# AI4Science-WestlakeU/safediffcon

Measured on AMD Instinct MI355X. Metric: sampled control trajectories/sec (1000-step DDPM), higher is better.
Workload: dtype f32; 1 GPU; C4: 2D smoke Unet3D_with_Conv3D dim=64 (1,2,4) state (B,32,7,64,64), B=64 per GPU, guided 1000-step DDPM, conformal quantile on; batch_per_gpu=64, global_batch=64, step=U-Net + guidance + posterior update of the whole batch, one hipGraph replay, parallelism=batch-sharded x1, no data-path collective, conv_precision=fp32

## Files before the change

include/sdc.h:

```cpp
#ifndef SDC_H
#define SDC_H

#include <stddef.h>
#include <stdint.h>

#ifdef __cplusplus
extern "C" {
#endif

#define SDC_OK 0
#define SDC_EINVAL (-1)
#define SDC_EALIGN (-2)
#define SDC_EHIP (-3)
#define SDC_ENULL (-4)

int sdc_version(void);
int sdc_last_error(char* buf, size_t cap);

typedef struct SdcConvDesc {
    int32_t B, Cin0, Cin1, Cout;
    int32_t iD, iH, iW;
    int32_t oD, oH, oW;
    int32_t kD, kH, kW;
    int32_t sD, sH, sW;
// ... 128 lines not shown
int sdc_burgers_rollout(const float* u0, const float* f, float* traj, int N, int s, int Nt, int steps, int record_every,
                        float dt, float coef_transport, float d0, float d1, float d2, void* stream);


typedef struct SdcWgradDesc {
    int32_t B, M, N;
    int32_t oD, oH, oW;
    int32_t iD, iH, iW;
    int32_t kD, kH, kW;
    int32_t sD, sH, sW;
    int32_t pD, pH, pW;
    int32_t uD, uH, uW;
    int32_t precision;
    int64_t gs[5], xs[5];
} SdcWgradDesc;
size_t sdc_conv_wgrad_bytes(const SdcWgradDesc* d);
int sdc_conv_wgrad(const SdcWgradDesc* d, const float* g, const float* x, float* dw, float* dbias, void* work,
                   size_t work_bytes, void* stream);

#define SDC_F16_EXP_INTS 1025
int sdc_f16_grad_exponent(const float* g, int B, int C, int D, int H, int W, const int64_t* strides, int32_t* e, void* stream);

int sdc_conv_dgrad_f16(const SdcConvDesc* d, const float* g, const float* wp, const int32_t* e, float* dx, void* stream);

size_t sdc_conv_wgrad_f16_bytes(const SdcWgradDesc* d);
int sdc_conv_wgrad_f16(const SdcWgradDesc* d, const float* g, const float* x, const int32_t* e, float* dw, float* dbias, void* work,
                       size_t work_bytes, void* stream);
int sdc_conv_wgrad_describe(const SdcWgradDesc* d, char* name, size_t cap);

int sdc_conv_stem_f16_ok(const SdcConvDesc* d);
size_t sdc_pack_stem_f16_bytes(int Cout, int Cin, int kD, int kH, int kW);
int sdc_pack_stem_f16(const float* w, void* out, int Cout, int Cin, int kD, int kH, int kW, void* stream);
int sdc_conv_stem_f16(const SdcConvDesc* d, const float* x, const void* wh, const float* bias, float* y, void* stream);

int sdc_conv_stem_x3_ok(const SdcConvDesc* d);
size_t sdc_pack_stem_x3_bytes(int Cout, int Cin, int kD, int kH, int kW);
int sdc_pack_stem_x3(const float* w, void* out, int Cout, int Cin, int kD, int kH, int kW, void* stream);
int sdc_conv_stem_x3(const SdcConvDesc* d, const float* x, const void* wb, const float* bias, float* y, void* stream);

int sdc_conv_gemm_x3_ok(const SdcConvDesc* d);
size_t sdc_pack_gemm_x3_bytes(int Cout, int Cin, int kH, int kW);
int sdc_pack_gemm_x3(const float* wp, void* out, int Cout, int Cin, int kH, int kW, void* stream);
int sdc_conv_gemm_x3(const SdcConvDesc* d, const float* x, const void* wb, const float* bias, float* y, void* stream);

int sdc_conv_pw_x3_ok(const SdcConvDesc* d);
int sdc_conv_pw_x3(const SdcConvDesc* d, const float* x0, const float* x1, const float* wp, const float* bias, const float* residual,
                   float* y, void* stream);

int sdc_conv_wino3_x3_ok(const SdcConvDesc* d);
size_t sdc_pack_wino3_x3_bytes(int Cout, int Cin);
int sdc_pack_wino3_x3(const float* wp, void* out, int Cout, int Cin, void* stream);
int sdc_conv_wino3_x3(const SdcConvDesc* d, const float* x, const float* x1, const void* wb, const float* bias, float* y,
                      double* gn_parts, int gn_groups, void* stream);

size_t sdc_gn_silu_bwd_floats(int B, int C, int G, int64_t S);
int sdc_gn_silu_bwd(const float* h, const float* gy, const float* stats, const float* gamma, const float* beta,
                    const float* ss, int64_t ss_b_stride, float* rows, float* gh, float* dgamma, float* dbeta, float* dss,
                    int B, int C, int G, int64_t S, void* stream);

size_t sdc_chan_norm_bwd_parts(int B, int64_t S);
size_t sdc_chan_norm_bwd_bytes(int B, int C, int64_t S);
int sdc_chan_norm_bwd(const float* x, const float* gy, const float* g, float* gx, float* gpart, int B, int C, int64_t S,
                      int mode, float eps, void* stream);

size_t sdc_pack_conv_weight_floats(int Cout, int Cin, int kD, int kH, int kW, int precision);
int sdc_pack_conv_weight(const float* w, float* out, int Cout, int Cin, int kD, int kH, int kW, int precision, int flip, void* stream);

typedef struct SdcPackItem {
    const float* w;
    float* out;
    int Cout, Cin, kD, kH, kW, precision, flip;
    int co_sh, ci_sh, grid_x, grid_y, block0;
    unsigned tap_magic;
    int64_t n[5];
} SdcPackItem;
int sdc_pack_batch_plan(SdcPackItem* items, int n, int* total_blocks, int* lds_bytes);
int sdc_pack_batch_run(const SdcPackItem* items_dev, int n, int total_blocks, int lds_bytes, void* stream);

size_t sdc_attn_bwd_bytes(int outer, int inner, int heads, int ntok);
int sdc_attn_bwd(const float* qkv, const float* dout, const float* rot, const float* bias, float* dqkv, float* dbias, void* work,
                 int outer, int inner, int heads, int ntok, int64_t q_so, int64_t q_sc, int64_t q_si, int64_t q_st,
                 int64_t o_so, int64_t o_sc, int64_t o_si, int64_t o_st, void* stream);

size_t sdc_tattn_block_bwd_bytes(int outer, int inner);
int sdc_tattn_block_bwd(const float* x, const float* g_pre, const float* wqkv, const float* wo, const float* rot, const float* bias,
                        const float* dy, float* dx, float* dg, float* dwqkv, float* dwo, float* dbias, void* work,
                        int outer, int inner, int C, int ntok, int64_t so, int64_t sc, int64_t st, float eps, void* stream);
size_t sdc_linattn_bwd_bytes(int outer, int inner, int heads, int64_t n);
int sdc_linattn_bwd(const float* qkv, const float* dout, float* dqkv, void* work, int outer, int inner, int heads, int64_t n,
                    int64_t q_so, int64_t q_sc, int64_t q_si, int64_t o_so, int64_t o_sc, int64_t o_si, void* stream);

int sdc_act_bwd(const float* x, const float* gy, float* gx, int64_t n, int kind, void* stream);

int sdc_sumpool2(const float* g, float* gx, int64_t rows, int H, int W, int fh, int fw, void* stream);

int sdc_linear(const float* x, const float* w, const float* bias, float* y, int rows, int K, int M, int64_t x_stride,
               int64_t y_stride, void* stream);
int sdc_linear_dgrad(const float* gy, const float* w, float* gx, int rows, int K, int M, int64_t gy_stride, int64_t gx_stride,
                     void* stream);
int sdc_linear_wgrad(const float* gy, const float* x, float* gw, float* gbias, int rows, int K, int M, int64_t gy_stride,
                     int64_t x_stride, void* stream);

typedef struct {
    const void* ptr;
    int64_t nwords;
} SdcSpan;
// ... 87 lines not shown
```

safediffcon_amd/_lib.py:

```python
import ctypes as C
import os

_HERE = os.path.dirname(os.path.abspath(__file__))
LIB_PATH = os.path.join(_HERE, "libsdc_hip.so")

SDC_MODEL_BURGERS, SDC_MODEL_TOKAMAK, SDC_MODEL_SMOKE = 0, 1, 2

_f32p = C.c_void_p
_i32p = C.c_void_p
_stream = C.c_void_p
_i64 = C.c_int64


class SdcConvDesc(C.Structure):
    _fields_ = [(n, C.c_int32) for n in (
        "B", "Cin0", "Cin1", "Cout", "iD", "iH", "iW", "oD", "oH", "oW", "kD", "kH", "kW", "sD", "sH", "sW",
        "pD", "pH", "pW", "uD", "uH", "uW", "up_mode", "precision")] + [
        ("x0s", C.c_int64 * 5), ("x1s", C.c_int64 * 5), ("ys", C.c_int64 * 5), ("rs", C.c_int64 * 5)]


class SdcStepDesc(C.Structure):
    _fields_ = [(n, C.c_int32) for n in (
        "model", "B", "d0", "d1", "d2", "d3", "guide", "clip", "impose", "cond_idx", "pad_zero", "use_max",
        "has_wgt", "skip_draws", "ddim")] + [("_pad", C.c_int32), ("seed", C.c_uint64)]
# ... 71 lines not shown
    "sdc_linattn_block_f16_bytes": (C.c_size_t, [C.c_int, C.c_int, C.c_int, _i64]),
    "sdc_linattn_block_f16": (C.c_int, [_f32p, _f32p, _f32p, _f32p, C.c_void_p, _f32p, _f32p, C.c_void_p, _f32p, C.c_int, C.c_int,
                                        C.c_int, _i64, _i64, _i64, _i64, C.c_int, C.c_int, C.c_float, _stream]),
    "sdc_linattn_block_gn_f16": (C.c_int, [_f32p, _f32p, _f32p, _f32p, C.c_int, _f32p, _f32p, _f32p, _f32p, C.c_void_p, _f32p, _f32p,
                                           C.c_void_p, _f32p, C.c_int, C.c_int, C.c_int, _i64, _i64, _i64, _i64, C.c_int, C.c_int,
                                           C.c_float, _stream]),
    "sdc_linattn_block_f16_ok": (C.c_int, [C.c_int, _i64]),
    "sdc_tattn_block": (C.c_int, [_f32p, _f32p, _f32p, _f32p, _f32p, _f32p, _f32p, C.c_int, C.c_int, C.c_int, C.c_int,
                                  _i64, _i64, _i64, C.c_float, _stream]),
    "sdc_pack_tattn_f16_bytes": (C.c_size_t, []),
    "sdc_pack_tattn_f16": (C.c_int, [_f32p, _f32p, C.c_void_p, _stream]),
    "sdc_tattn_block_f16": (C.c_int, [_f32p, _f32p, C.c_void_p, _f32p, _f32p, _f32p, C.c_int, C.c_int, C.c_int, C.c_int,
                                      _i64, _i64, _i64, C.c_float, _stream]),
    "sdc_pack_tattn_x3_bytes": (C.c_size_t, []),
    "sdc_pack_tattn_x3": (C.c_int, [_f32p, _f32p, C.c_void_p, _stream]),
    "sdc_tattn_block_x3": (C.c_int, [_f32p, _f32p, C.c_void_p, _f32p, _f32p, _f32p, C.c_int, C.c_int, C.c_int, C.c_int,
                                     _i64, _i64, _i64, C.c_float, _stream]),
    "sdc_tattn_block_x3_ok": (C.c_int, [C.c_int, C.c_int, C.c_int]),
    "sdc_attn": (C.c_int, [_f32p, _f32p, _f32p, _f32p, C.c_int, C.c_int, C.c_int, C.c_int, _i64, _i64, _i64, _i64,
                           _i64, _i64, _i64, _i64, _stream]),
    "sdc_act": (C.c_int, [_f32p, _f32p, _i64, C.c_int, _stream]),
    "sdc_guide_reduce": (C.c_int, [C.POINTER(SdcStepDesc), _f32p, _f32p, _f32p, _i32p, _f32p, _f32p, _stream]),
    "sdc_step_update": (C.c_int, [C.POINTER(SdcStepDesc), _f32p, _f32p, _f32p, _f32p, _i32p, _i32p, _f32p, _i64,
                                  _f32p, _f32p, _f32p, _f32p, _f32p, _f32p, _f32p, _f32p, _stream]),
    "sdc_impose": (C.c_int, [C.POINTER(SdcStepDesc), _f32p, _f32p, _f32p, _f32p, _stream]),
    "sdc_randn": (C.c_int, [_f32p, _i64, C.c_uint64, _i32p, _stream]),
    "sdc_advance": (C.c_int, [_i32p, C.c_int, _i32p, C.c_int, _stream]),
    "sdc_advance_table": (C.c_int, [_i32p, _i32p, _i32p, _i32p, C.c_int, _stream]),
    "sdc_conformal_score": (C.c_int, [C.POINTER(SdcStepDesc), _f32p, _f32p, _f32p, _f32p, _f32p, _f32p, _stream]),
    "sdc_burgers_rollout": (C.c_int, [_f32p, _f32p, _f32p, C.c_int, C.c_int, C.c_int, C.c_int, C.c_int, C.c_float, C.c_float,
                                      C.c_float, C.c_float, C.c_float, _stream]),
    "sdc_conv_wgrad_bytes": (C.c_size_t, [C.POINTER(SdcWgradDesc)]),
    "sdc_conv_wgrad": (C.c_int, [C.POINTER(SdcWgradDesc), _f32p, _f32p, _f32p, _f32p, C.c_void_p, C.c_size_t, _stream]),
    "sdc_f16_grad_exponent": (C.c_int, [_f32p, C.c_int, C.c_int, C.c_int, C.c_int, C.c_int, C.c_void_p, C.c_void_p, _stream]),
    "sdc_conv_dgrad_f16": (C.c_int, [C.POINTER(SdcConvDesc), _f32p, _f32p, C.c_void_p, _f32p, _stream]),
    "sdc_conv_stem_f16_ok": (C.c_int, [C.POINTER(SdcConvDesc)]),
    "sdc_pack_stem_f16_bytes": (C.c_size_t, [C.c_int, C.c_int, C.c_int, C.c_int, C.c_int]),
    "sdc_pack_stem_f16": (C.c_int, [_f32p, C.c_void_p, C.c_int, C.c_int, C.c_int, C.c_int, C.c_int, _stream]),
    "sdc_conv_stem_f16": (C.c_int, [C.POINTER(SdcConvDesc), _f32p, C.c_void_p, _f32p, _f32p, _stream]),
    "sdc_conv_stem_x3_ok": (C.c_int, [C.POINTER(SdcConvDesc)]),
    "sdc_pack_stem_x3_bytes": (C.c_size_t, [C.c_int, C.c_int, C.c_int, C.c_int, C.c_int]),
    "sdc_pack_stem_x3": (C.c_int, [_f32p, C.c_void_p, C.c_int, C.c_int, C.c_int, C.c_int, C.c_int, _stream]),
    "sdc_conv_stem_x3": (C.c_int, [C.POINTER(SdcConvDesc), _f32p, C.c_void_p, _f32p, _f32p, _stream]),
    "sdc_conv_gemm_x3_ok": (C.c_int, [C.POINTER(SdcConvDesc)]),
    "sdc_pack_gemm_x3_bytes": (C.c_size_t, [C.c_int, C.c_int, C.c_int, C.c_int]),
    "sdc_pack_gemm_x3": (C.c_int, [_f32p, C.c_void_p, C.c_int, C.c_int, C.c_int, C.c_int, _stream]),
    "sdc_conv_gemm_x3": (C.c_int, [C.POINTER(SdcConvDesc), _f32p, C.c_void_p, _f32p, _f32p, _stream]),
    "sdc_conv_pw_x3_ok": (C.c_int, [C.POINTER(SdcConvDesc)]),
    "sdc_conv_pw_x3": (C.c_int, [C.POINTER(SdcConvDesc), _f32p, _f32p, _f32p, _f32p, _f32p, _f32p, _stream]),
    "sdc_conv_wino3_x3_ok": (C.c_int, [C.POINTER(SdcConvDesc)]),
    "sdc_pack_wino3_x3_bytes": (C.c_size_t, [C.c_int, C.c_int]),
    "sdc_pack_wino3_x3": (C.c_int, [_f32p, C.c_void_p, C.c_int, C.c_int, _stream]),
    "sdc_conv_wino3_x3": (C.c_int, [C.POINTER(SdcConvDesc), _f32p, _f32p, C.c_void_p, _f32p, _f32p, C.c_void_p, C.c_int, _stream]),
    "sdc_conv_wgrad_f16_bytes": (C.c_size_t, [C.POINTER(SdcWgradDesc)]),
    "sdc_conv_wgrad_f16": (C.c_int, [C.POINTER(SdcWgradDesc), _f32p, _f32p, C.c_void_p, _f32p, _f32p, C.c_void_p, C.c_size_t, _stream]),
    "sdc_conv_wgrad_describe": (C.c_int, [C.POINTER(SdcWgradDesc), C.c_char_p, C.c_size_t]),
    "sdc_gn_silu_bwd_floats": (C.c_size_t, [C.c_int, C.c_int, C.c_int, _i64]),
    "sdc_gn_silu_bwd": (C.c_int, [_f32p, _f32p, _f32p, _f32p, _f32p, _f32p, _i64, _f32p, _f32p, _f32p, _f32p, _f32p,
                                  C.c_int, C.c_int, C.c_int, _i64, _stream]),
    "sdc_chan_norm_bwd_parts": (C.c_size_t, [C.c_int, _i64]),
    "sdc_chan_norm_bwd_bytes": (C.c_size_t, [C.c_int, C.c_int, _i64]),
    "sdc_chan_norm_bwd": (C.c_int, [_f32p, _f32p, _f32p, _f32p, _f32p, C.c_int, C.c_int, _i64, C.c_int, C.c_float, _stream]),
    "sdc_pack_conv_weight_floats": (C.c_size_t, [C.c_int, C.c_int, C.c_int, C.c_int, C.c_int, C.c_int]),
    "sdc_pack_conv_weight": (C.c_int, [_f32p, _f32p, C.c_int, C.c_int, C.c_int, C.c_int, C.c_int, C.c_int, C.c_int, _stream]),
    "sdc_pack_batch_plan": (C.c_int, [C.POINTER(SdcPackItem), C.c_int, C.POINTER(C.c_int), C.POINTER(C.c_int)]),
    "sdc_pack_batch_run": (C.c_int, [C.c_void_p, C.c_int, C.c_int, C.c_int, _stream]),
    "sdc_tattn_block_bwd_bytes": (C.c_size_t, [C.c_int, C.c_int]),
    "sdc_tattn_block_bwd": (C.c_int, [_f32p, _f32p, _f32p, _f32p, _f32p, _f32p, _f32p, _f32p, _f32p, _f32p, _f32p, _f32p, C.c_void_p,
                                      C.c_int, C.c_int, C.c_int, C.c_int, _i64, _i64, _i64, C.c_float, _stream]),
    "sdc_attn_bwd_bytes": (C.c_size_t, [C.c_int, C.c_int, C.c_int, C.c_int]),
    "sdc_attn_bwd": (C.c_int, [_f32p, _f32p, _f32p, _f32p, _f32p, _f32p, C.c_void_p, C.c_int, C.c_int, C.c_int, C.c_int,
                               _i64, _i64, _i64, _i64, _i64, _i64, _i64, _i64, _stream]),
    "sdc_linattn_bwd_bytes": (C.c_size_t, [C.c_int, C.c_int, C.c_int, _i64]),
    "sdc_linattn_bwd": (C.c_int, [_f32p, _f32p, _f32p, C.c_void_p, C.c_int, C.c_int, C.c_int, _i64, _i64, _i64, _i64, _i64, _i64, _i64,
                                  _stream]),
    "sdc_act_bwd": (C.c_int, [_f32p, _f32p, _f32p, _i64, C.c_int, _stream]),
    "sdc_sumpool2": (C.c_int, [_f32p, _f32p, _i64, C.c_int, C.c_int, C.c_int, C.c_int, _stream]),
    "sdc_kstar_lstm_floats": (C.c_size_t, []),
    "sdc_kstar_rollout": (C.c_int, [C.POINTER(SdcKstarModel), _f32p, _i64, _i64, _i64, C.c_void_p, C.c_void_p, C.c_int, C.c_int, _stream]),
    "sdc_smoke_rollout_workspace_bytes": (C.c_size_t, [C.c_int]),
    "sdc_smoke_rollout": (C.c_int, [_f32p, _f32p, _i64, _i64, _f32p, _i64, _f32p, _i64, C.c_void_p, C.c_void_p, C.c_void_p,
                                    C.c_int, C.c_int, C.c_void_p, C.c_void_p, C.c_void_p, C.c_size_t, C.c_int, C.c_int, C.c_int,
                                    C.c_int, C.c_int, C.c_int, C.c_double, C.c_int, _stream]),
    "sdc_conv_splitk_bytes": (C.c_size_t, [C.POINTER(SdcConvDesc)]),
    "sdc_conv_splitk": (C.c_int, [C.POINTER(SdcConvDesc), _f32p, _f32p, _f32p, _f32p, _f32p, _f32p, C.c_size_t, _stream]),
    "sdc_linear": (C.c_int, [_f32p, _f32p, _f32p, _f32p, C.c_int, C.c_int, C.c_int, _i64, _i64, _stream]),
    "sdc_linear_dgrad": (C.c_int, [_f32p, _f32p, _f32p, C.c_int, C.c_int, C.c_int, _i64, _i64, _stream]),
    "sdc_linear_wgrad": (C.c_int, [_f32p, _f32p, _f32p, _f32p, C.c_int, C.c_int, C.c_int, _i64, _i64, _stream]),
    "sdc_checksum_spans": (C.c_int, [C.c_void_p, C.c_int, C.c_void_p, _stream]),
    "sdc_optim_plan": (C.c_int, [C.POINTER(SdcOptItem), C.c_int, C.c_int, C.POINTER(C.c_int), C.POINTER(C.c_int), C.POINTER(C.c_int)]),
    "sdc_optim_bytes": (C.c_size_t, [C.c_int]),
    "sdc_optim_step": (C.c_int, [C.c_int, C.c_void_p, C.c_int, C.c_int, C.c_int, C.c_int, C.c_void_p, C.c_void_p, C.c_void_p, C.c_int,
                                 _stream]),
    "sdc_graph_begin": (C.c_int, [_stream]),
    "sdc_graph_end": (C.c_int, [_stream, C.POINTER(C.c_void_p)]),
    "sdc_graph_launch": (C.c_int, [C.c_void_p, _stream]),
    "sdc_graph_destroy": (C.c_int, [C.c_void_p]),
    "sdc_event_create": (C.c_int, [C.POINTER(C.c_void_p)]),
    "sdc_event_record": (C.c_int, [C.c_void_p, _stream]),
    "sdc_event_elapsed_ms": (C.c_int, [C.c_void_p, C.c_void_p, C.POINTER(C.c_float)]),
    "sdc_event_destroy": (C.c_int, [C.c_void_p]),
}

_lib = None


# ... 36 lines not shown
```

safediffcon_amd/build.py:

```python
import os
import subprocess
import sys

HERE = os.path.dirname(os.path.abspath(__file__))
CSRC = os.path.join(HERE, "csrc")
LIB = os.path.join(HERE, "libsdc_hip.so")
SOURCES = ["sdc_api.hip", "sdc_conv.hip", "sdc_conv_wino.hip", "sdc_conv_f16.hip", "sdc_conv_stem_f16.hip", "sdc_conv_stem_x3.hip", "sdc_conv_gemm_x3.hip", "sdc_conv_pw_x3.hip", "sdc_conv_wino_x3.hip", "sdc_norm.hip", "sdc_attn.hip", "sdc_lablock.hip", "sdc_lablock_f16.hip", "sdc_lablock_x3.hip", "sdc_tablock.hip", "sdc_tablock_f16.hip", "sdc_tablock_x3.hip", "sdc_tablock_bwd.hip", "sdc_step.hip", "sdc_solver.hip", "sdc_grad.hip", "sdc_wgrad_f16.hip", "sdc_attn_bwd.hip", "sdc_kstar.hip", "sdc_smoke.hip", "sdc_linear.hip", "sdc_optim.hip"]
HEADERS = ["sdc_common.h", "sdc_lablock_tile.h", "sdc_tablock_tile.h", "sdc_conv_stem_tile.h", "sdc_split3.h", "sdc_f16frag.h", "sdc_conv.h", "sdc_conv_wino3s.inc", "sdc_conv_wino2s.inc", "sdc_conv_pw2.inc"]
HIPCC = os.environ.get("HIPCC", "/opt/rocm/bin/hipcc")
FLAGS = ["--offload-arch=gfx950", "-O3", "-fPIC", "-std=c++17", "-Wall", "-Wno-unused-function"]


def source_hash():
    import hashlib
    h = hashlib.sha256()
    for f in SOURCES + HEADERS:
        with open(os.path.join(CSRC, f), "rb") as fh:
            h.update(fh.read())
    with open(os.path.join(HERE, "..", "include", "sdc.h"), "rb") as fh:
        h.update(fh.read())
    return h.hexdigest()[:16]


def _stale(out, deps):
    if not os.path.exists(out):
        return True
    t = os.path.getmtime(out)
    return any(os.path.getmtime(d) > t for d in deps)


def build_experiments(verbose=True):
    out = os.path.join(HERE, "libsdc_hip_exp.so")
    cmd = [HIPCC, *FLAGS, "-DSDC_KERNEL_EXPERIMENTS", "-shared", *[os.path.join(CSRC, s) for s in SOURCES], "-o", out]
    if verbose:
        print(" ".join(cmd), flush=True)
    subprocess.check_call(cmd)
    return out


def build(force=False, verbose=True, jobs=4):
    from concurrent.futures import ThreadPoolExecutor
    hdrs = [os.path.join(CSRC, h) for h in HEADERS] + [os.path.join(HERE, "..", "include", "sdc.h")]
    objs, todo = [], []
    for src in SOURCES:
        s = os.path.join(CSRC, src)
        o = os.path.join(CSRC, src.replace(".hip", ".o"))
        if force or _stale(o, [s] + hdrs):
            todo.append([HIPCC, *FLAGS, "-c", s, "-o", o])
        objs.append(o)

    def run(cmd):
        if verbose:
            print(" ".join(cmd), flush=True)
        subprocess.check_call(cmd)
    if todo:
        with ThreadPoolExecutor(max_workers=max(1, min(jobs, len(todo)))) as ex:
            list(ex.map(run, todo))
    if force or _stale(LIB, objs):
        run([HIPCC, "--offload-arch=gfx950", "-shared", "-fPIC", *objs, "-o", LIB])
    return LIB

# ... 7 lines not shown
```

safediffcon_amd/csrc/sdc_conv_wino_x3.hip:

```cpp
#include "sdc_conv.h"
#include "sdc_split3.h"

using namespace sdcconv;

namespace {

typedef __bf16 bf16x4 __attribute__((ext_vector_type(4)));
typedef float w2f2 __attribute__((ext_vector_type(2)));
typedef float nfloat4 __attribute__((ext_vector_type(4)));
typedef float nfloat2 __attribute__((ext_vector_type(2)));

__device__ __forceinline__ w2f2 pk_add2(w2f2 a, w2f2 b) { w2f2 r; asm("v_pk_add_f32 %0, %1, %2" : "=v"(r) : "v"(a), "v"(b)); return r; }
__device__ __forceinline__ w2f2 pk_sub2(w2f2 a, w2f2 b) { w2f2 r; asm("v_pk_add_f32 %0, %1, %2 neg_lo:[0,1] neg_hi:[0,1]" : "=v"(r) : "v"(a), "v"(b)); return r; }
__device__ __forceinline__ w2f2 pk_fma2(w2f2 a, w2f2 b, w2f2 c) { w2f2 r; asm("v_pk_fma_f32 %0, %1, %2, %3" : "=v"(r) : "v"(a), "v"(b), "v"(c)); return r; }
__device__ __forceinline__ w2f2 pk_fms2(w2f2 a, w2f2 b, w2f2 c) { w2f2 r; asm("v_pk_fma_f32 %0, %1, %2, %3 neg_lo:[0,0,1] neg_hi:[0,0,1]" : "=v"(r) : "v"(a), "v"(b), "v"(c)); return r; }
__device__ __forceinline__ w2f2 pk_fnma2(w2f2 a, w2f2 b, w2f2 c) { w2f2 r; asm("v_pk_fma_f32 %0, %1, %2, %3 neg_lo:[0,1,0] neg_hi:[0,1,0]" : "=v"(r) : "v"(a), "v"(b), "v"(c)); return r; }
__device__ __forceinline__ w2f2 pk_sumdiff(w2f2 c) {
    w2f2 r;
    asm("v_pk_add_f32 %0, %1, %1 op_sel:[0,1] op_sel_hi:[1,0] neg_hi:[0,1]" : "=v"(r) : "v"(c));
    return r;
}
__device__ __forceinline__ w2f2 pk_sumdiff_fwd(w2f2 c) {
    w2f2 r;
    asm("v_pk_add_f32 %0, %1, %1 op_sel:[0,1] op_sel_hi:[0,1] neg_hi:[0,1]" : "=v"(r) : "v"(c));
// ... 406 lines not shown
            const int idx = a.gn_cpg >= BM ? ntl * (a.gn_cpg / BM) + (m0 - g * a.gn_cpg) / BM : ntl;
            double* pp = a.gn_part + (((int64_t)ob * a.gn_G + g) * a.gn_nparts + idx) * 2;
            pp[0] = sum; pp[1] = sq;
        }
    }
}

__global__ __launch_bounds__(256) void pack_wino3_x3_kernel(const float* __restrict__ u3, __bf16* __restrict__ out, int Cout, int Cin, int64_t n) {
    const int64_t e = (int64_t)blockIdx.x * 256 + threadIdx.x;
    if (e >= n) return;
    const int c16 = (int)(e & 15), col = (int)((e >> 4) & 63), xi = (int)((e >> 10) & 3), j = (int)((e >> 12) & 3);
    int64_t r = e >> 14;
    const int S1 = Cin / 16;
    const int st = (int)(r % S1); r /= S1;
    const int jd = (int)(r & 3);
    const int mt = (int)(r >> 2);
    const int ci = st * 16 + (c16 ^ (((col >> 3) & 1) << 3)), co = mt * 64 + col;
    __bf16 ph, pm, pl;
    split3(u3[(((int64_t)jd * Cin + ci) * Cout + co) * 16 + j * 4 + xi], ph, pm, pl);
    out[e] = ph; out[n + e] = pm; out[2 * n + e] = pl;
}

bool x3_small(const SdcConvDesc& d) {
    auto span = [](const int64_t* st, int b, int dd, int h, int w) {
        return (int64_t)(b - 1) * st[0] + (int64_t)(dd - 1) * st[2] + (int64_t)(h - 1) * st[3] + (int64_t)(w - 1) * st[4];
    };
    return span(d.x0s, d.B, d.iD, d.iH, d.iW) < (1ll << 30) && (d.Cin1 == 0 || span(d.x1s, d.B, d.iD, d.iH, d.iW) < (1ll << 30));
}

bool wino3_x3_covers(const SdcConvDesc& d) {
    if (!(d.B > 0 && d.Cin0 > 0 && d.Cin1 >= 0 && d.Cout > 0 && d.oW == 16)) return false;
    if (d.Cin0 % X3_SK != 0 || d.Cin1 % X3_SK != 0) return false;
    SdcConvDesc e = d;
    e.precision = 4;
    if (!wg3_ok(e, x3_small(e))) return false;
    return (int64_t)64 * (d.Cin0 + d.Cin1) * d.Cout * 2 < (1ll << 30);
}

int wino3_x3_gnparts(const SdcConvDesc& d, int G) {
    if (G <= 0 || d.Cout % G) return 0;
    const int cpg = d.Cout / G;
    const int64_t S = (int64_t)d.oD * d.oH * d.oW;
    const int bn = X3_TILES * 8;
    if (cpg % 8 || S % bn || !(cpg % X3_BM == 0 || X3_BM % cpg == 0)) return 0;
    return (int)(S / bn) * (cpg >= X3_BM ? cpg / X3_BM : 1);
}

bool wino3_x3_faster(const SdcConvDesc& d) {
    if (!(d.oD == 32 && d.oH == 16 && d.oW == 16)) return false;
    const int c0 = d.Cin0, c1 = d.Cin1, co = d.Cout;
    return (c0 == 128 && c1 == 0 && co == 256) || (c0 == 256 && c1 == 0 && co == 256) || (c0 == 256 && c1 == 256 && co == 128);
}

}

extern "C" int sdc_conv_wino3_x3_ok(const SdcConvDesc* dp) {
    return dp && wino3_x3_covers(*dp) && wino3_x3_faster(*dp) ? 1 : 0;
}

extern "C" size_t sdc_pack_wino3_x3_bytes(int Cout, int Cin) {
    if (Cout <= 0 || Cout % 64 != 0 || Cin <= 0 || Cin % 16 != 0) return 0;
    return (size_t)3 * 64 * Cin * Cout * sizeof(__bf16);
}

extern "C" int sdc_pack_wino3_x3(const float* wp, void* out, int Cout, int Cin, void* stream) {
    SDC_REQUIRE(wp && out, SDC_ENULL, "sdc_pack_wino3_x3: null pointer");
    SDC_REQUIRE(sdc_pack_wino3_x3_bytes(Cout, Cin) > 0, SDC_EINVAL, "sdc_pack_wino3_x3: Cout a multiple of 64, Cin a multiple of 16 (got Cin %d, Cout %d)", Cin, Cout);
    const int64_t n = (int64_t)64 * Cin * Cout;
    SDC_REQUIRE(n / 256 + 1 < (1ll << 31), SDC_EINVAL, "sdc_pack_wino3_x3: weight too large");
    const int64_t K = (int64_t)27 * Cin;
    const float* u3 = wp + K * Cout + (K / 3 * 4) * Cout + (K / 9 * 16) * Cout;
    hipLaunchKernelGGL(pack_wino3_x3_kernel, dim3((unsigned)((n + 255) / 256)), dim3(256), 0, sdc::as_stream(stream), u3,
                       reinterpret_cast<__bf16*>(out), Cout, Cin, n);
    return sdc::check_launch("sdc_pack_wino3_x3");
}

extern "C" int sdc_conv_wino3_x3(const SdcConvDesc* dp, const float* x, const float* x1, const void* wb, const float* bias, float* y,
                                 double* gn_parts, int gn_groups, void* stream) {
    SDC_REQUIRE(dp && x && wb && y, SDC_ENULL, "sdc_conv_wino3_x3: null pointer");
    const SdcConvDesc& d = *dp;
    SDC_REQUIRE(d.Cin1 <= 0 || x1, SDC_ENULL, "sdc_conv_wino3_x3: Cin1 > 0 but x1 is null");
    SDC_REQUIRE(wino3_x3_covers(d), SDC_EINVAL, "sdc_conv_wino3_x3: descriptor not covered: %dx%dx%d taps, stride %dx%dx%d, Cin %d+%d, Cout %d, "
                "residual %d, output %dx%dx%d", d.kD, d.kH, d.kW, d.sD, d.sH, d.sW, d.Cin0, d.Cin1, d.Cout, (int)(d.rs[1] != 0), d.oD, d.oH, d.oW);
    auto al = [](const void* p, int b) { return reinterpret_cast<uintptr_t>(p) % b == 0; };
    SDC_REQUIRE(al(wb, 16) && al(x, 8) && (d.Cin1 == 0 || al(x1, 8)) && al(y, 8), SDC_EALIGN,
                "sdc_conv_wino3_x3: the packed weight buffer must be 16-byte aligned, x, x1 and y 8-byte aligned");
    WinoX3Args a;
    a.d = d;
    a.x0 = x; a.x1 = x1; a.wb = reinterpret_cast<const __bf16*>(wb); a.bias = bias; a.y = y;
    a.Cin = d.Cin0 + d.Cin1;
    a.plane_bytes = (uint32_t)((int64_t)64 * a.Cin * d.Cout * 2);
    a.gn_part = nullptr; a.gn_G = a.gn_cpg = a.gn_nparts = 0;
    if (gn_parts) {
        const int np = wino3_x3_gnparts(d, gn_groups);
        SDC_REQUIRE(np > 0, SDC_EINVAL, "sdc_conv_wino3_x3: shape not covered by the fused statistics (%d groups over %d channels)", gn_groups, d.Cout);
        a.gn_part = gn_parts; a.gn_G = gn_groups; a.gn_cpg = d.Cout / gn_groups; a.gn_nparts = np;
    }
    const int64_t tiles = (int64_t)d.B * (d.oD / 2) * (d.oH / 2) * (d.oW / 2);
    const dim3 grid((unsigned)((tiles / X3_TILES) * (d.Cout / X3_BM)));
#define X3_LAUNCH(D)                                                                                             \
    do {                                                                                                         \
        static std::atomic<uint64_t> attr{0};                                                                    \
        SDC_LDS_OPTIN(attr, (conv_wg3_x3_kernel<16, D>), 160 * 1024, "sdc_conv_wino3_x3");                       \
        hipLaunchKernelGGL((conv_wg3_x3_kernel<16, D>), grid, dim3(256), X3_LDS, sdc::as_stream(stream), a);     \
    } while (0)
#ifdef SDC_KERNEL_EXPERIMENTS
    static const int dbg = exp_env("SDC_WG3X_DBG");
    switch (dbg) {
        case 0: break;
        case 1: X3_LAUNCH(1); return sdc::check_launch("sdc_conv_wino3_x3"); case 2: X3_LAUNCH(2); return sdc::check_launch("sdc_conv_wino3_x3");
        case 4: X3_LAUNCH(4); return sdc::check_launch("sdc_conv_wino3_x3"); case 8: X3_LAUNCH(8); return sdc::check_launch("sdc_conv_wino3_x3");
        case 16: X3_LAUNCH(16); return sdc::check_launch("sdc_conv_wino3_x3"); case 32: X3_LAUNCH(32); return sdc::check_launch("sdc_conv_wino3_x3");
        case 64: X3_LAUNCH(64); return sdc::check_launch("sdc_conv_wino3_x3"); case 6: X3_LAUNCH(6); return sdc::check_launch("sdc_conv_wino3_x3");
        case 15: X3_LAUNCH(15); return sdc::check_launch("sdc_conv_wino3_x3"); case 31: X3_LAUNCH(31); return sdc::check_launch("sdc_conv_wino3_x3");
        default: X3_LAUNCH(63); return sdc::check_launch("sdc_conv_wino3_x3");
    }
#endif
    X3_LAUNCH(0);
#undef X3_LAUNCH
    return sdc::check_launch("sdc_conv_wino3_x3");
}
```

Baseline: 0.3086 trajectories/s.

## Add wide 128-channel Winograd x3 conv kernel for mid-resolution layers

Adds a second Winograd 3x3 split-bf16 convolution kernel that covers 128 output channels per workgroup instead of 64. It loops over two halves of the spatial tile so each transformed weight block loaded into LDS is reused across more outputs. The default entry point now picks this wide form automatically for three 32x16x16 layer shapes. In exchange it uses more LDS and registers per workgroup (one wave per EU), launches half as many workgroups, and duplicates a large kernel body that could hide indexing bugs.

Measured after the change: 0.3115 trajectories/s (median of 6 runs). Within noise of the previous version (+0.9%).

```diff
diff --git a/include/sdc.h b/include/sdc.h
--- a/include/sdc.h
+++ b/include/sdc.h
@@ -204,6 +204,10 @@
 int sdc_pack_wino3_x3(const float* wp, void* out, int Cout, int Cin, void* stream);
 int sdc_conv_wino3_x3(const SdcConvDesc* d, const float* x, const float* x1, const void* wb, const float* bias, float* y,
                       double* gn_parts, int gn_groups, void* stream);
+
+int sdc_conv_wino3_x3_wide_ok(const SdcConvDesc* d);
+int sdc_conv_wino3_x3_sel(const SdcConvDesc* d, const float* x, const float* x1, const void* wb, const float* bias, float* y,
+                          double* gn_parts, int gn_groups, int impl, void* stream);
 
 size_t sdc_gn_silu_bwd_floats(int B, int C, int G, int64_t S);
 int sdc_gn_silu_bwd(const float* h, const float* gy, const float* stats, const float* gamma, const float* beta,
diff --git a/safediffcon_amd/_lib.py b/safediffcon_amd/_lib.py
--- a/safediffcon_amd/_lib.py
+++ b/safediffcon_amd/_lib.py
@@ -147,6 +147,8 @@
     "sdc_pack_wino3_x3_bytes": (C.c_size_t, [C.c_int, C.c_int]),
     "sdc_pack_wino3_x3": (C.c_int, [_f32p, C.c_void_p, C.c_int, C.c_int, _stream]),
     "sdc_conv_wino3_x3": (C.c_int, [C.POINTER(SdcConvDesc), _f32p, _f32p, C.c_void_p, _f32p, _f32p, C.c_void_p, C.c_int, _stream]),
+    "sdc_conv_wino3_x3_wide_ok": (C.c_int, [C.POINTER(SdcConvDesc)]),
+    "sdc_conv_wino3_x3_sel": (C.c_int, [C.POINTER(SdcConvDesc), _f32p, _f32p, C.c_void_p, _f32p, _f32p, C.c_void_p, C.c_int, C.c_int, _stream]),
     "sdc_conv_wgrad_f16_bytes": (C.c_size_t, [C.POINTER(SdcWgradDesc)]),
     "sdc_conv_wgrad_f16": (C.c_int, [C.POINTER(SdcWgradDesc), _f32p, _f32p, C.c_void_p, _f32p, _f32p, C.c_void_p, C.c_size_t, _stream]),
     "sdc_conv_wgrad_describe": (C.c_int, [C.POINTER(SdcWgradDesc), C.c_char_p, C.c_size_t]),
diff --git a/safediffcon_amd/build.py b/safediffcon_amd/build.py
--- a/safediffcon_amd/build.py
+++ b/safediffcon_amd/build.py
@@ -6,7 +6,7 @@
 CSRC = os.path.join(HERE, "csrc")
 LIB = os.path.join(HERE, "libsdc_hip.so")
 SOURCES = ["sdc_api.hip", "sdc_conv.hip", "sdc_conv_wino.hip", "sdc_conv_f16.hip", "sdc_conv_stem_f16.hip", "sdc_conv_stem_x3.hip", "sdc_conv_gemm_x3.hip", "sdc_conv_pw_x3.hip", "sdc_conv_wino_x3.hip", "sdc_norm.hip", "sdc_attn.hip", "sdc_lablock.hip", "sdc_lablock_f16.hip", "sdc_lablock_x3.hip", "sdc_tablock.hip", "sdc_tablock_f16.hip", "sdc_tablock_x3.hip", "sdc_tablock_bwd.hip", "sdc_step.hip", "sdc_solver.hip", "sdc_grad.hip", "sdc_wgrad_f16.hip", "sdc_attn_bwd.hip", "sdc_kstar.hip", "sdc_smoke.hip", "sdc_linear.hip", "sdc_optim.hip"]
-HEADERS = ["sdc_common.h", "sdc_lablock_tile.h", "sdc_tablock_tile.h", "sdc_conv_stem_tile.h", "sdc_split3.h", "sdc_f16frag.h", "sdc_conv.h", "sdc_conv_wino3s.inc", "sdc_conv_wino2s.inc", "sdc_conv_pw2.inc"]
+HEADERS = ["sdc_common.h", "sdc_lablock_tile.h", "sdc_tablock_tile.h", "sdc_conv_stem_tile.h", "sdc_split3.h", "sdc_f16frag.h", "sdc_conv.h", "sdc_conv_wino3s.inc", "sdc_conv_wino2s.inc", "sdc_conv_pw2.inc", "sdc_conv_wino3x_wide.inc"]
 HIPCC = os.environ.get("HIPCC", "/opt/rocm/bin/hipcc")
 FLAGS = ["--offload-arch=gfx950", "-O3", "-fPIC", "-std=c++17", "-Wall", "-Wno-unused-function"]
 
diff --git a/safediffcon_amd/csrc/sdc_conv_wino3x_wide.inc b/safediffcon_amd/csrc/sdc_conv_wino3x_wide.inc
--- /dev/null
+++ b/safediffcon_amd/csrc/sdc_conv_wino3x_wide.inc
@@ -0,0 +1,387 @@
+constexpr int XW_BM = 128, XW_HT = 32;
+constexpr int XW_UPC = 4 * XW_BM * X3_SK * 2;
+constexpr int XW_UIMG = 3 * XW_UPC;
+constexpr int XW_VPC = 4 * XW_HT * X3_SK * 2;
+constexpr int XW_VIMG = 3 * XW_VPC;
+constexpr int XW_U = 0, XW_V = 2 * XW_UIMG;
+constexpr int XW_SCR = XW_V + 2 * XW_VIMG;
+constexpr int XW_STASH = XW_SCR + 2 * 4 * 8 * 8;
+constexpr int XW_LDS = XW_STASH + 256 * 8 * 4;
+
+template <int OW, int DBG = 0>
+__global__ __launch_bounds__(256) __attribute__((amdgpu_waves_per_eu(1))) void conv_wg3_x3w_kernel(const WinoX3Args a) {
+    static_assert(OW == 16, "rows of 16: one lane per tile and stage channel pair");
+    constexpr int TW = OW / 2, LGW = 4;
+    typedef const __attribute__((address_space(1))) char* gchar_p;
+    typedef const __attribute__((address_space(1))) nfloat2* gfloat2_p;
+    typedef unsigned int u32x4 __attribute__((ext_vector_type(4)));
+    typedef const __attribute__((address_space(1))) u32x4* guint4_p;
+    typedef __attribute__((address_space(1))) char* gwchar_p;
+    typedef __attribute__((address_space(1))) nfloat2* gwfloat2_p;
+    extern __shared__ __attribute__((aligned(16))) char lds[];
+
+    const SdcConvDesc& d = a.d;
+    const int wave = SDC_UNIFORM(threadIdx.x >> 6);
+    const int MT = d.Cout / XW_BM;
+    const int lb = xcd_tile(blockIdx.x, gridDim.x);
+    const int mt = lb % MT;
+    const int m0 = mt * XW_BM;
+    const int tile0 = (lb / MT) * X3_TILES;
+    const int H2 = d.oH >> 1, D2 = d.oD >> 1;
+    int ob, od, hp0;
+    {
+        const int rp0 = tile0 >> (LGW - 1);
+        const int q = (int)(((float)rp0 + 0.5f) * (1.0f / (float)H2));
+        const int b = (int)(((float)q + 0.5f) * (1.0f / (float)D2));
+        hp0 = SDC_UNIFORM(rp0 - q * H2);
+        ob = SDC_UNIFORM(b);
+        od = SDC_UNIFORM(2 * (q - b * D2));
+    }
+    const bool two = d.Cin1 > 0;
+
+    const int64_t xs1_0 = d.x0s[1], xs1_1 = d.x1s[1];
+    const int cin0 = d.Cin0, cin = a.Cin;
+    const int S1 = cin / X3_SK;
+    const uint32_t ublock = (uint32_t)S1 * (16u * X3_RUN * 2u);
+    const float* const x0p = a.x0 + (int64_t)ob * d.x0s[0] + (int64_t)od * d.x0s[2];
+    const float* const x1p = two ? a.x1 + (int64_t)ob * d.x1s[0] + (int64_t)od * d.x1s[2] : x0p;
+    const int64_t xs2_0 = d.x0s[2], xs2_1 = two ? d.x1s[2] : d.x0s[2];
+    const uint32_t lo_u = (uint32_t)(-od) >> 31, hi_u = (uint32_t)(od + 2 - d.iD) >> 31;
+    const bool gn = a.gn_part != nullptr;
+
+    f32x16 zero16;
+#pragma unroll
+    for (int r = 0; r < 16; ++r) zero16[r] = 0.0f;
+
+#pragma unroll 1
+    for (int half = 0; half < 2; ++half) {
+        int tid = threadIdx.x;
+        asm volatile("" : "+v"(tid));
+        asm volatile("" : "+s"(ob));
+        const int lane = tid & 63;
+        const int l31 = lane & 31, lh = lane >> 5;
+        const int prl = 2 * (l31 >> 4) + (lane & 1), pc0 = 2 * ((lane & 15) >> 1);
+        const int ptile = prl * TW + (pc0 >> 1);
+        const int cp = wave * 2 + lh;
+        const int vpark = XW_V + ptile * 32 + (((cp >> 2) ^ ((ptile >> 3) & 1)) * 16) + (cp & 3) * 4;
+        const int afrag = XW_U + (wave >> 1) * (XW_UPC / 2) + ((wave & 1) * 32 + l31) * 32 + (lh ^ ((l31 >> 3) & 1)) * 16;
+        const int bfrag = XW_V + l31 * 32 + (lh ^ ((l31 >> 3) & 1)) * 16;
+        uint32_t uoffv = (uint32_t)tid * 16u, uoffv1 = uoffv + 4096u;
+
+        const int hp = hp0 + 4 * half + prl;
+        const bool up_ok = hp > 0, dn_ok = 2 * hp + 2 < d.iH;
+        const uint32_t rsel0 = up_ok ? OW * 4 : 0, rsel3 = dn_ok ? 2 * OW * 4 : 0;
+        const uint32_t vp = (uint32_t)((2 * hp) * OW + pc0) * 4u;
+
+        w2f2 raw[2][2][4];
+        int s_jd = 0, s_ci = 0;
+        float mka = 0.f, mkb = 0.f;
+        const float *f_xa = x0p, *f_xb = x0p;
+        int64_t f_sc = 0;
+        uint32_t voff = vp, voff0 = vp - rsel0, voff3 = vp + rsel3;
+        auto fetch_raw_begin = [&]() __attribute__((always_inline)) {
+            const bool first = s_ci < cin0;
+            f_sc = first ? xs1_0 : xs1_1;
+            const int64_t xs2 = first ? xs2_0 : xs2_1;
+            const int cbase = (first ? s_ci : s_ci - cin0) + wave * 4;
+            const float* bsel = (first ? x0p : x1p) + (int64_t)cbase * f_sc;
+            voff = vp + (uint32_t)lh * 8u * (uint32_t)f_sc;
+            voff0 = voff - rsel0;
+            voff3 = voff + rsel3;
+            const int jd_u = SDC_UNIFORM(s_jd);
+            const uint32_t j0 = (uint32_t)((jd_u ^ 2) - 1) >> 31, j2 = (uint32_t)((jd_u ^ 1) - 1) >> 31, j3 = (uint32_t)((jd_u ^ 3) - 1) >> 31;
+            const int da = -(int)(j0 & lo_u);
+            const int db = 1 + (int)j3 * (2 * (int)hi_u - 1);
+            mka = __builtin_bit_cast(float, (0x3F800000u & ((j0 & (lo_u ^ 1u)) - 1u)) | (j2 << 31));
+            mkb = __builtin_bit_cast(float, (0x3F800000u & ((j3 & (hi_u ^ 1u)) - 1u)) | ((j0 | (j3 & hi_u)) << 31));
+            f_xa = bsel + da * xs2;
+            f_xb = bsel + db * xs2;
+            const int nci = s_ci + X3_SK;
+            const bool wrap = nci >= cin;
+            s_ci = wrap ? 0 : nci;
+            s_jd = wrap ? ((s_jd + 1) & 3) : s_jd;
+        };
+        auto fetch_raw_rows = [&](int ch, int sl) __attribute__((always_inline)) {
+            const gchar_p rb = (gchar_p)uniform_ptr((sl ? f_xb : f_xa) + ch * f_sc);
+            asm volatile("" : "+v"(voff), "+v"(voff0), "+v"(voff3));
+            const nfloat2 v0 = *(gfloat2_p)(rb + voff0), v1 = *(gfloat2_p)(rb + voff), v2 = *(gfloat2_p)(rb + voff + OW * 4), v3 = *(gfloat2_p)(rb + voff3);
+            raw[ch][sl][0] = w2f2{v0.x, v0.y}; raw[ch][sl][1] = w2f2{v1.x, v1.y};
+            raw[ch][sl][2] = w2f2{v2.x, v2.y}; raw[ch][sl][3] = w2f2{v3.x, v3.y};
+        };
+        w2f2 hrow[2][4];
+        w2f2 ka0, kb0, ka3, kb3;
+        auto h_begin = [&](float ca, float cb) __attribute__((always_inline)) {
+            const float f0 = rsel0 ? 1.0f : 0.0f, f3 = rsel3 ? 1.0f : 0.0f;
+            const w2f2 m0p = {f0, f0}, m3p = {f3, f3};
+            ka0 = pks_mul(m0p, ca); kb0 = pks_mul(m0p, cb); ka3 = pks_mul(m3p, ca); kb3 = pks_mul(m3p, cb);
+        };
+        auto h_transform = [&](int ch, float ca, float cb) __attribute__((always_inline)) {
+            const w2f2 e1 = pks_fma(raw[ch][1][1], cb, pks_mul(raw[ch][0][1], ca));
+            const w2f2 e2 = pks_fma(raw[ch][1][2], cb, pks_mul(raw[ch][0][2], ca));
+            hrow[ch][0] = pk_fma2(raw[ch][1][0], kb0, pk_fms2(raw[ch][0][0], ka0, e2));
+            hrow[ch][1] = pk_add2(e1, e2);
+            hrow[ch][2] = pk_sub2(e2, e1);
+            hrow[ch][3] = pk_fnma2(raw[ch][1][3], kb3, pk_fnma2(raw[ch][0][3], ka3, e1));
+        };
+        float px[2], pf[2];
+        uint32_t ph = 0, pm = 0, pl = 0;
+        w2f2 sdv[2];
+        auto park_step = [&](int buf, int j, int xi, int k) __attribute__((always_inline)) {
+#pragma clang fp contract(off)
+            if (k == 0) {
+#pragma unroll
+                for (int ch = 0; ch < 2; ++ch) {
+                    const w2f2 cc = hrow[ch][j];
+                    if (xi == 0) px[ch] = sub_prev2(cc.y, cc.y);
+                    else if (xi == 1) { sdv[ch] = pk_sumdiff(cc); px[ch] = sdv[ch].x; }
+                    else if (xi == 2) px[ch] = sdv[ch].y;
+                    else px[ch] = sub_next2(cc.x, cc.x);
+                }
+                ph = cvt_pk_bf16(px[0], px[1]);
+            } else if (k == 1) {
+                pf[0] = bf16_lo(ph); pf[1] = bf16_hi(ph);
+#pragma unroll
+                for (int i = 0; i < 2; ++i) px[i] = px[i] - pf[i];
+            } else if (k == 2) {
+                pm = cvt_pk_bf16(px[0], px[1]);
+                pf[0] = bf16_lo(pm); pf[1] = bf16_hi(pm);
+            } else if (k == 3) {
+#pragma unroll
+                for (int i = 0; i < 2; ++i) px[i] = px[i] - pf[i];
+                pl = cvt_pk_bf16(px[0], px[1]);
+            } else {
+                char* dst = lds + vpark + buf * XW_VIMG + xi * 1024;
+                *reinterpret_cast<uint32_t*>(dst) = ph;
+                *reinterpret_cast<uint32_t*>(dst + XW_VPC) = pm;
+                *reinterpret_cast<uint32_t*>(dst + 2 * XW_VPC) = pl;
+            }
+        };
+        u32x4 ureg[12];
+        int u_p = 0, u_st = 0, u_j = 0;
+        gchar_p u_base = (gchar_p)uniform_ptr(reinterpret_cast<const float*>(a.wb));
+        auto fetch_u_begin = [&]() __attribute__((always_inline)) {
+            const int jdc = (0xC9 >> (2 * u_p)) & 3;
+            const int run = ((mt * 8 + jdc) * S1 + u_st) * 4 + u_j;
+            u_base = (gchar_p)uniform_ptr(reinterpret_cast<const float*>(a.wb + (int64_t)run * X3_RUN));
+            const bool wj = u_j == 3, ws = wj && u_st + 1 == S1;
+            u_j = (u_j + 1) & 3;
+            u_st = ws ? 0 : (wj ? u_st + 1 : u_st);
+            u_p = ws ? ((u_p + 1) & 3) : u_p;
+        };
+        auto fetch_u_item = [&](int k) __attribute__((always_inline)) {
+            asm volatile("" : "+v"(uoffv), "+v"(uoffv1));
+            const gchar_p b = u_base + (uint32_t)((uint32_t)(k >> 2) * a.plane_bytes + (uint32_t)((k >> 1) & 1) * ublock);
+            ureg[k] = *(guint4_p)(b + ((k & 1) ? uoffv1 : uoffv));
+        };
+        auto park_u_item = [&](int buf, int k) __attribute__((always_inline)) {
+            *reinterpret_cast<u32x4*>(lds + XW_U + buf * XW_UIMG + 4096 * k + uoffv) = ureg[k];
+        };
+        bf16x8 fr[2][6];
+        auto read_frag = [&](int buf, int xi, int set, int p) __attribute__((always_inline)) {
+            fr[set][p] = p < 3 ? *reinterpret_cast<const bf16x8*>(lds + afrag + buf * XW_UIMG + p * XW_UPC + xi * 2048)
+                               : *reinterpret_cast<const bf16x8*>(lds + bfrag + buf * XW_VIMG + (p - 3) * XW_VPC + xi * 1024);
+        };
+
+        f32x16 acc[16];
+        {
+            const float* bp = a.bias;
+            asm volatile("" : "+s"(bp));
+            if (bp) {
+                bp += m0 + wave * 32 + 4 * lh;
+#pragma unroll
+                for (int r = 0; r < 16; ++r) acc[5][r] = bp[8 * (r >> 2) + (r & 3)];
+            } else {
+                acc[5] = zero16;
+            }
+        }
+        float pka, pkb;
+        {
+            fetch_raw_begin();
+            pka = mka; pkb = mkb;
+#pragma unroll
+            for (int g = 0; g < 4; ++g) fetch_raw_rows(g >> 1, g & 1);
+            fetch_u_begin();
+#pragma unroll
+            for (int k = 0; k < 12; ++k) fetch_u_item(k);
+            h_begin(pka, pkb);
+#pragma unroll
+            for (int ch = 0; ch < 2; ++ch) h_transform(ch, pka, pkb);
+#pragma unroll
+            for (int k = 0; k < 12; ++k) park_u_item(0, k);
+#pragma unroll
+            for (int st = 0; st < 20; ++st) park_step(0, 0, st / 5, st % 5);
+            fetch_u_begin();
+#pragma unroll
+            for (int k = 0; k < 12; ++k) fetch_u_item(k);
+        }
+        __syncthreads();
+#pragma unroll
+        for (int p = 0; p < 6; ++p) read_frag(0, 0, 0, p);
+
+        const int cob = m0 + wave * 32;
+        const int nloc = half * XW_HT + l31;
+        const int ohp = hp0 + (nloc >> (LGW - 1)), otw = nloc & (TW - 1);
+        const uint32_t yoff = (uint32_t)((2 * ohp) * d.ys[3] + (2 * otw) * d.ys[4] + (4 * lh) * d.ys[1]) * 4u;
+        const uint32_t yoff1 = yoff + (uint32_t)d.ys[3] * 4u;
+        float gp[8];
+        float* const gstash = reinterpret_cast<float*>(lds + XW_STASH + 2 * uoffv);
+
+        auto fold = [&](const int p) __attribute__((always_inline)) {
+            const bool t0 = p == 1 || p == 2, t1 = p != 2;
+            const bool ld0 = p == 2, ld1 = p == 1 || p == 3;
+            const bool fin0 = p == 2, fin1 = p == 3;
+            const bool always = d.Cout > 0;
+            const int LEAD = 2;
+            const int64_t ycs4 = d.ys[1] * 4;
+            float* const y0p = a.y + (int64_t)ob * d.ys[0] + (int64_t)od * d.ys[2] + (int64_t)cob * d.ys[1];
+            gwchar_p s0 = (gwchar_p)(__attribute__((address_space(1))) void*)uniform_ptr(y0p);
+            gwchar_p s1 = (gwchar_p)(__attribute__((address_space(1))) void*)uniform_ptr(y0p + d.ys[2]);
+            gchar_p l0 = (gchar_p)s0, l1 = (gchar_p)s1;
+            w2f2 P0[4][4][2], P1[4][4][2];
+            auto load_block = [&](int g4) __attribute__((always_inline)) {
+#pragma unroll
+                for (int r3 = 0; r3 < 4; ++r3) {
+                    if (ld0) { P0[g4][r3][0] = *(gfloat2_p)(l0 + yoff); P0[g4][r3][1] = *(gfloat2_p)(l0 + yoff1); l0 += r3 < 3 ? ycs4 : 5 * ycs4; }
+                    if (ld1) { P1[g4][r3][0] = *(gfloat2_p)(l1 + yoff); P1[g4][r3][1] = *(gfloat2_p)(l1 + yoff1); l1 += r3 < 3 ? ycs4 : 5 * ycs4; }
+                }
+            };
+            if (ld0 || ld1) {
+#pragma unroll
+                for (int g = 0; g < LEAD; ++g) load_block(g);
+            }
+#pragma unroll
+            for (int g4 = 0; g4 < 4; ++g4) {
+                if (g4 + LEAD < 4 && (ld0 || ld1)) load_block(g4 + LEAD);
+                if (!always) continue;
+                w2f2 bs2 = {0.f, 0.f}, bq2 = {0.f, 0.f};
+#pragma unroll
+                for (int r3 = 0; r3 < 4; ++r3) {
+                    const int rr = g4 * 4 + r3;
+                    w2f2 pa[4], pb[4];
+#pragma unroll
+                    for (int j = 0; j < 4; ++j) {
+                        pa[j] = w2f2{acc[4 * j][rr], acc[4 * j + 3][rr]};
+                        pb[j] = w2f2{acc[4 * j + 1][rr], acc[4 * j + 2][rr]};
+                    }
+                    const w2f2 t0a = pk_add2(pk_add2(pa[0], pa[1]), pa[2]), t1a = pk_sub2(pk_sub2(pa[1], pa[2]), pa[3]);
+                    const w2f2 t0b = pk_add2(pk_add2(pb[0], pb[1]), pb[2]), t1b = pk_sub2(pk_sub2(pb[1], pb[2]), pb[3]);
+                    const w2f2 z0 = pk_addsub(pk_sumdiff_fwd(t0b), t0a);
+                    const w2f2 z1 = pk_addsub(pk_sumdiff_fwd(t1b), t1a);
+                    if (t0) {
+                        const bool have = p == 1 ? ld1 : ld0;
+                        const w2f2 b0 = p == 1 ? P1[g4][r3][0] : P0[g4][r3][0], b1 = p == 1 ? P1[g4][r3][1] : P0[g4][r3][1];
+                        const w2f2 u0 = have ? pk_add2(b0, z0) : z0, u1 = have ? pk_add2(b1, z1) : z1;
+                        *(gwfloat2_p)(s0 + yoff) = nfloat2{u0.x, u0.y};
+                        *(gwfloat2_p)(s0 + yoff1) = nfloat2{u1.x, u1.y};
+                        s0 += r3 < 3 ? ycs4 : 5 * ycs4;
+                        if (fin0) { bs2 = pk_add2(bs2, pk_add2(u0, u1)); bq2 = pk_sqacc(u1, pk_sqacc(u0, bq2)); }
+                    }
+                    if (t1) {
+                        const w2f2 u0 = ld1 ? pk_sub2(P1[g4][r3][0], z0) : z0, u1 = ld1 ? pk_sub2(P1[g4][r3][1], z1) : z1;
+                        *(gwfloat2_p)(s1 + yoff) = nfloat2{u0.x, u0.y};
+                        *(gwfloat2_p)(s1 + yoff1) = nfloat2{u1.x, u1.y};
+                        s1 += r3 < 3 ? ycs4 : 5 * ycs4;
+                        if (fin1) { bs2 = pk_add2(bs2, pk_add2(u0, u1)); bq2 = pk_sqacc(u1, pk_sqacc(u0, bq2)); }
+                    }
+                }
+                if (fin0 || fin1) { gp[2 * g4] = bs2.x + bs2.y; gp[2 * g4 + 1] = bq2.x + bq2.y; }
+            }
+            if (fin0 && gn) {
+                *reinterpret_cast<nfloat4*>(gstash) = nfloat4{gp[0], gp[1], gp[2], gp[3]};
+                *reinterpret_cast<nfloat4*>(gstash + 4) = nfloat4{gp[4], gp[5], gp[6], gp[7]};
+            }
+        };
+
+        auto substage = [&](auto FIRST, auto J, const int pass) __attribute__((always_inline)) {
+            constexpr bool first = decltype(FIRST)::value;
+            constexpr int j = decltype(J)::value;
+            constexpr int rbuf = j & 1, wbuf = rbuf ^ 1, jn = (j + 1) & 3;
+#pragma unroll
+            for (int sl = 0; sl < 24; ++sl) {
+                const int xi = sl / 6, t = sl % 6, c = 4 * j + xi, set = xi & 1;
+                const f32x16 cstart = (first && t == 0) ? ((c == 5 && pass == 0) ? acc[5] : zero16) : acc[c];
+                acc[c] = __builtin_amdgcn_mfma_f32_32x32x16_bf16(fr[set][X3_PA[t]], fr[set][3 + X3_PB[t]], cstart, 0, 0, 0);
+                if (xi < 3) read_frag(rbuf, xi + 1, set ^ 1, t);
+                else if (t >= 3) { read_frag(wbuf, 0, 0, 2 * (t - 3)); read_frag(wbuf, 0, 0, 2 * (t - 3) + 1); }
+                if (sl < 12 && !(DBG & 4)) park_u_item(wbuf, sl);
+                if (sl >= 1 && sl < 13) { if (sl == 1) fetch_u_begin(); if (!(DBG & 2)) fetch_u_item(sl - 1); }
+                if (sl < 20 && !(DBG & 1)) park_step(wbuf, jn, sl / 5, sl % 5);
+                if (j == 0 && sl >= 12 && sl < 16 && !(DBG & 8)) {
+                    if (sl == 12) { fetch_raw_begin(); pka = mka; pkb = mkb; }
+                    fetch_raw_rows((sl - 12) >> 1, (sl - 12) & 1);
+                }
+                if (j == 2 && sl >= 22) {
+                    if (sl == 22) h_begin(pka, pkb);
+                    h_transform(sl - 22, pka, pkb);
+                }
+                __builtin_amdgcn_sched_barrier(0);
+                if (sl == 20) __syncthreads();
+            }
+        };
+        auto stage = [&](auto FIRST, const int pass) __attribute__((always_inline)) {
+            substage(FIRST, std::integral_constant<int, 0>{}, pass);
+            substage(FIRST, std::integral_constant<int, 1>{}, pass);
+            substage(FIRST, std::integral_constant<int, 2>{}, pass);
+            substage(FIRST, std::integral_constant<int, 3>{}, pass);
+        };
+        auto run_pass = [&](auto P) __attribute__((always_inline)) {
+            constexpr int p = decltype(P)::value;
+            stage(std::true_type{}, p);
+            for (int st = 1; st < S1; ++st) stage(std::false_type{}, p);
+            fold(p);
+#pragma unroll
+            for (int q = 0; q < 6; ++q) read_frag(0, 0, 0, q);
+        };
+        run_pass(std::integral_constant<int, 0>{});
+        run_pass(std::integral_constant<int, 1>{});
+        run_pass(std::integral_constant<int, 2>{});
+        run_pass(std::integral_constant<int, 3>{});
+
+        if (gn) {
+            double gv[8];
+            const nfloat4 s0 = *reinterpret_cast<const nfloat4*>(gstash), s1 = *reinterpret_cast<const nfloat4*>(gstash + 4);
+            const float g0[8] = {s0.x, s0.y, s0.z, s0.w, s1.x, s1.y, s1.z, s1.w};
+#pragma unroll
+            for (int i = 0; i < 8; ++i) gv[i] = (double)g0[i] + (double)gp[i];
+            const double tot = wave_sum8(gv, lane);
+            if ((lane & 7) == 0) reinterpret_cast<double*>(lds + XW_SCR)[(half * 4 + wave) * 8 + (lane >> 3)] = tot;
+        }
+    }
+
+    if (gn) {
+        const int tid = threadIdx.x;
+        const double* scr = reinterpret_cast<const double*>(lds + XW_SCR);
+        __syncthreads();
+        const int BM = X3_BM;
+        const int ngl = a.gn_cpg >= BM ? 1 : BM / a.gn_cpg;
+        if (tid < 2 * ngl) {
+            const int cb = tid / ngl, t = tid - cb * ngl;
+            const int mb = m0 + cb * BM;
+            const int r0 = a.gn_cpg >= BM ? 0 : t * a.gn_cpg, r1 = a.gn_cpg >= BM ? BM : r0 + a.gn_cpg;
+            double sum = 0.0, sq = 0.0;
+            for (int blk = r0 / 8; blk < r1 / 8; ++blk) {
+                const int wv = cb * 2 + (blk >> 2), k = blk & 3;
+                for (int h = 0; h < 2; ++h) {
+                    sum += scr[((h * 4 + wv) * 4 + k) * 2];
+                    sq += scr[((h * 4 + wv) * 4 + k) * 2 + 1];
+                }
+            }
+            const int g = (mb + r0) / a.gn_cpg;
+            const int ntl = tile0 / X3_TILES - ob * (D2 * H2 * TW / X3_TILES);
+            const int idx = a.gn_cpg >= BM ? ntl * (a.gn_cpg / BM) + (mb - g * a.gn_cpg) / BM : ntl;
+            double* pp = a.gn_part + (((int64_t)ob * a.gn_G + g) * a.gn_nparts + idx) * 2;
+            pp[0] = sum; pp[1] = sq;
+        }
+    }
+}
+
+bool wino3_x3_wide_covers(const SdcConvDesc& d) {
+    if (!wino3_x3_covers(d) || d.Cout % XW_BM != 0) return false;
+    return d.x0s[1] >= 0 && d.x0s[1] < (1ll << 27) && (d.Cin1 == 0 || (d.x1s[1] >= 0 && d.x1s[1] < (1ll << 27)));
+}
+
+bool wino3_x3_wide_faster(const SdcConvDesc& d) {
+    if (!(d.oD == 32 && d.oH == 16 && d.oW == 16)) return false;
+    const int c0 = d.Cin0, c1 = d.Cin1, co = d.Cout;
+    return (c0 == 128 && c1 == 0 && co == 256) || (c0 == 256 && c1 == 0 && co == 256) || (c0 == 256 && c1 == 256 && co == 128);
+}
diff --git a/safediffcon_amd/csrc/sdc_conv_wino_x3.hip b/safediffcon_amd/csrc/sdc_conv_wino_x3.hip
--- a/safediffcon_amd/csrc/sdc_conv_wino_x3.hip
+++ b/safediffcon_amd/csrc/sdc_conv_wino_x3.hip
@@ -482,6 +482,8 @@
     return (c0 == 128 && c1 == 0 && co == 256) || (c0 == 256 && c1 == 0 && co == 256) || (c0 == 256 && c1 == 256 && co == 128);
 }
 
+#include "sdc_conv_wino3x_wide.inc"
+
 }
 
 extern "C" int sdc_conv_wino3_x3_ok(const SdcConvDesc* dp) {
@@ -505,13 +507,25 @@
     return sdc::check_launch("sdc_pack_wino3_x3");
 }
 
+extern "C" int sdc_conv_wino3_x3_wide_ok(const SdcConvDesc* dp) {
+    return dp && wino3_x3_wide_covers(*dp) && wino3_x3_faster(*dp) && wino3_x3_wide_faster(*dp) ? 1 : 0;
+}
+
 extern "C" int sdc_conv_wino3_x3(const SdcConvDesc* dp, const float* x, const float* x1, const void* wb, const float* bias, float* y,
                                  double* gn_parts, int gn_groups, void* stream) {
+    return sdc_conv_wino3_x3_sel(dp, x, x1, wb, bias, y, gn_parts, gn_groups, sdc_conv_wino3_x3_wide_ok(dp), stream);
+}
+
+extern "C" int sdc_conv_wino3_x3_sel(const SdcConvDesc* dp, const float* x, const float* x1, const void* wb, const float* bias, float* y,
+                                     double* gn_parts, int gn_groups, int impl, void* stream) {
     SDC_REQUIRE(dp && x && wb && y, SDC_ENULL, "sdc_conv_wino3_x3: null pointer");
+    SDC_REQUIRE(impl == 0 || impl == 1, SDC_EINVAL, "sdc_conv_wino3_x3_sel: impl %d (0: narrow form, 1: wide form)", impl);
     const SdcConvDesc& d = *dp;
     SDC_REQUIRE(d.Cin1 <= 0 || x1, SDC_ENULL, "sdc_conv_wino3_x3: Cin1 > 0 but x1 is null");
     SDC_REQUIRE(wino3_x3_covers(d), SDC_EINVAL, "sdc_conv_wino3_x3: descriptor not covered: %dx%dx%d taps, stride %dx%dx%d, Cin %d+%d, Cout %d, "
                 "residual %d, output %dx%dx%d", d.kD, d.kH, d.kW, d.sD, d.sH, d.sW, d.Cin0, d.Cin1, d.Cout, (int)(d.rs[1] != 0), d.oD, d.oH, d.oW);
+    SDC_REQUIRE(impl == 0 || wino3_x3_wide_covers(d), SDC_EINVAL, "sdc_conv_wino3_x3_sel: the wide form needs whole 128-channel blocks and "
+                "channel strides below 2^27 elements (Cout %d)", d.Cout);
     auto al = [](const void* p, int b) { return reinterpret_cast<uintptr_t>(p) % b == 0; };
     SDC_REQUIRE(al(wb, 16) && al(x, 8) && (d.Cin1 == 0 || al(x1, 8)) && al(y, 8), SDC_EALIGN,
                 "sdc_conv_wino3_x3: the packed weight buffer must be 16-byte aligned, x, x1 and y 8-byte aligned");
@@ -527,6 +541,28 @@
         a.gn_part = gn_parts; a.gn_G = gn_groups; a.gn_cpg = d.Cout / gn_groups; a.gn_nparts = np;
     }
     const int64_t tiles = (int64_t)d.B * (d.oD / 2) * (d.oH / 2) * (d.oW / 2);
+    if (impl == 1) {
+        const dim3 grid((unsigned)((tiles / X3_TILES) * (d.Cout / XW_BM)));
+#define X3W_LAUNCH(D)                                                                                             \
+    do {                                                                                                          \
+        static std::atomic<uint64_t> attr{0};                                                                     \
+        SDC_LDS_OPTIN(attr, (conv_wg3_x3w_kernel<16, D>), 160 * 1024, "sdc_conv_wino3_x3");                       \
+        hipLaunchKernelGGL((conv_wg3_x3w_kernel<16, D>), grid, dim3(256), XW_LDS, sdc::as_stream(stream), a);     \
+    } while (0)
+#ifdef SDC_KERNEL_EXPERIMENTS
+        static const int wdbg = exp_env("SDC_WG3X_DBG");
+        switch (wdbg) {
+            case 0: break;
+            case 1: X3W_LAUNCH(1); return sdc::check_launch("sdc_conv_wino3_x3"); case 2: X3W_LAUNCH(2); return sdc::check_launch("sdc_conv_wino3_x3");
+            case 4: X3W_LAUNCH(4); return sdc::check_launch("sdc_conv_wino3_x3"); case 8: X3W_LAUNCH(8); return sdc::check_launch("sdc_conv_wino3_x3");
+            case 6: X3W_LAUNCH(6); return sdc::check_launch("sdc_conv_wino3_x3");
+            default: X3W_LAUNCH(15); return sdc::check_launch("sdc_conv_wino3_x3");
+        }
+#endif
+        X3W_LAUNCH(0);
+#undef X3W_LAUNCH
+        return sdc::check_launch("sdc_conv_wino3_x3");
+    }
     const dim3 grid((unsigned)((tiles / X3_TILES) * (d.Cout / X3_BM)));
 #define X3_LAUNCH(D)                                                                                             \
     do {                                                                                                         \
```
